# openclimatefix/predict_pv_yield

Measured on AMD Instinct MI355X. Metric: PV-site samples/sec (train step), conv3d 12->6 frames, higher is better.
Workload: dtype bf16; 1 GPU; conv3d train step (fwd + NMAE + bwd + Adam): sat [B,11,18,64,64] N(0,1), 4x Conv3d(3x3x3, 32ch) + fc 128/128/64, 128.6 M params; per_gpu_batch=32, global_batch=32, t_frames=18, parallelism=single

## Files before the change

include/pv_yield_hip.h:

```cpp
#ifndef PV_YIELD_HIP_H
#define PV_YIELD_HIP_H

#include <stddef.h>
#include <stdint.h>

#ifdef __cplusplus
extern "C" {
#endif

#define PV_ABI_VERSION 1

enum {
  PV_OK = 0,
  PV_EINVAL = -1,
  PV_ESIZE = -2,
  PV_ELAUNCH = -3
};

enum { PV_BORDER_CONSTANT = 0, PV_BORDER_REPLICATE = 1 };

enum {
  PV_U8_ROUND_DIV4 = 0,
  PV_U8_TRUNC_SCALE = 1
};
// ... 195 lines not shown
                               int transpose_flip, void* stream);

#define PV_PACK_MAX_JOBS 16
typedef struct pv_pack_job {
  const float* w;
  uint16_t* wp;
  int32_t c_out, c_in, transpose_flip;
} pv_pack_job;
int pv_conv3d_pack_weights_multi_bf16(const pv_pack_job* jobs, int32_t n_jobs, void* stream);

int pv_relu_mask_dims(int32_t h, int32_t w, int32_t* hp, int32_t* wp);
int pv_conv3d_fwd_bf16(const uint16_t* x, const uint16_t* gate, const uint16_t* wp,
                       const float* bias, uint16_t* y, const uint16_t* out_gate,
                       const uint32_t* out_gate_mask, uint32_t* relu_mask_out,
                       const pv_conv3d_dims* d, int relu, int y_ncdhw, void* stream);

int pv_conv3d_fwd_bf16_f32in(const float* x, uint16_t* xp_out, const uint16_t* wp, const float* bias, uint16_t* y,
                             uint32_t* relu_mask_out, const pv_conv3d_dims* d, int relu, void* stream);

int pv_conv3d_bwd_weight_bf16_workspace_bytes(const pv_conv3d_dims* d, size_t* bytes);
int pv_conv3d_bwd_weight_bf16(const uint16_t* x, const uint16_t* dy, const uint16_t* y_relu_mask,
                              float* dw, float* dbias, const pv_conv3d_dims* d,
                              void* workspace, size_t workspace_bytes, void* stream);
int pv_conv3d_bwd_weight_f16(const uint16_t* x, const uint16_t* dy, float* dw, float* dbias, const pv_conv3d_dims* d,
                             void* workspace, size_t workspace_bytes, void* stream);

size_t pv_conv3d_split2_weight_elems(void);
int pv_conv3d_pack_weight_split2_f16(const float* w, uint16_t* wp, float* state, int32_t c_out, int32_t c_in, void* stream);
int pv_conv3d_fwd_f16_f32out(const uint16_t* x, const uint16_t* wp, void* y, int32_t y_is_f16, const pv_conv3d_dims* d, void* stream);
int pv_conv3d_fwd_f16_f32out_covers(const pv_conv3d_dims* d);
int pv_sum3_ndhwc_to_ncdhw_f32(const float* parts, const uint16_t* p01_f16, const float* sx_state, const float* sw_state,
                               int32_t data_gradient, const float* bias, const uint16_t* gate_h, float* y, uint16_t* out_h,
                               uint16_t* out_l, float* max_state, int32_t relu, int32_t batch, int64_t vox_per_sample, void* stream);

int pv_linear_f32_skinny_covers(int32_t m, int32_t n, int64_t k);
size_t pv_linear_fwd_f32_skinny_workspace_bytes(int32_t n);
int pv_linear_fwd_f32_skinny(const float* x, const float* w, const float* bias, float* y, int32_t m, int32_t n, int64_t k, int32_t relu,
                             void* workspace, size_t workspace_bytes, void* stream);
int pv_linear_dx_f32_skinny(const float* g, const float* w, float* dx, int32_t m, int32_t n, int64_t k, void* stream);

int pv_linear_workspace_bytes(int32_t m, int32_t n, int64_t k, size_t* bytes);
int pv_linear_fwd_f32(const float* x, const float* w, const float* bias, float* y,
                      int32_t m, int32_t n, int64_t k, int relu,
                      void* workspace, size_t workspace_bytes, void* stream);
int pv_linear_bwd_f32(const float* x, const float* w, const float* dy, const float* y_relu_mask,
                      float* dx, float* dw, float* db,
// ... 175 lines not shown
```

predict_pv_yield_amd/_lib.py:

```python
import ctypes
import os
import subprocess

_PKG = os.path.dirname(os.path.abspath(__file__))
LIB_PATH = os.environ.get("PV_YIELD_LIB") or os.path.join(_PKG, "lib", "libpvyield_hip.so")
CSRC_DIR = os.path.join(_PKG, "csrc")

PV_BORDER_CONSTANT = 0
PV_BORDER_REPLICATE = 1
PV_U8_ROUND_DIV4 = 0
PV_U8_TRUNC_SCALE = 1
PV_OPTFLOW_FARNEBACK_GAUSSIAN = 256

c_i32, c_i64, c_f32, c_f64 = ctypes.c_int32, ctypes.c_int64, ctypes.c_float, ctypes.c_double
c_vp, c_sz, c_int, c_u8 = ctypes.c_void_p, ctypes.c_size_t, ctypes.c_int, ctypes.c_uint8


class FarnebackParams(ctypes.Structure):
    _fields_ = [("pyr_scale", c_f64), ("levels", c_i32), ("winsize", c_i32), ("iterations", c_i32),
                ("poly_n", c_i32), ("poly_sigma", c_f64), ("flags", c_i32)]


class Conv3dDims(ctypes.Structure):
    _fields_ = [("batch", c_i32), ("c_in", c_i32), ("c_out", c_i32), ("t_in", c_i32), ("h_in", c_i32),
# ... 59 lines not shown
    "pv_u8_stacks_from_normalised_f32": [c_vp, c_i64, c_i64, c_i64, c_i64, c_vp, c_i64, c_i32, c_i32, c_i64, c_i32, c_f32, c_vp],
    "pv_remap_bilinear_nhwc_f32": [c_vp, c_i64, c_vp, c_i64, c_i64, c_vp, c_i64, c_i64, c_i64, c_i32, c_f32, c_i32, c_i32,
                                   c_i32, c_int, c_f32, c_vp],
    "pv_normalise_i16": [c_vp, c_vp, c_sz, c_i64, c_i32, c_vp, c_vp, c_vp],
    "pv_normalise_f32": [c_vp, c_vp, c_sz, c_i64, c_i32, c_vp, c_vp, c_vp],
    "pv_bf16_cpad": [c_i32],
    "pv_pack_ncdhw_f32_to_ndhwc_bf16": [c_vp, c_vp, c_i32, c_i32, c_i32, c_i32, c_i32, c_vp],
    "pv_pack_split2_ncdhw_f32_to_ndhwc_f16": [c_vp, c_vp, c_vp, c_vp, c_i32, c_i32, c_i32, c_i32, c_i32, c_i32, c_vp],
    "pv_unpack_ndhwc_bf16_to_ncdhw_f32": [c_vp, c_vp, c_i32, c_i32, c_i32, c_i32, c_i32, c_vp],
    "pv_repack_gate_ncdhw_to_ndhwc_bf16": [c_vp, c_vp, c_vp, c_i32, c_i32, c_i32, c_i32, c_i32, c_vp],
    "pv_conv3d_packed_weight_elems": [c_i32],
    "pv_conv3d_pack_weight_bf16": [c_vp, c_vp, c_i32, c_i32, c_int, c_vp],
    "pv_relu_mask_dims": [c_i32, c_i32, c_vp, c_vp],
    "pv_ssim_mean_u8": [c_vp, c_i64, c_vp, c_i64, c_i64, c_i32, c_i32, c_f64, c_vp, c_vp],
    "pv_ssim_mean_f32": [c_vp, c_i64, c_vp, c_i64, c_i64, c_i32, c_i32, c_f64, c_vp, c_vp],
    "pv_stage_timing_begin": [],
    "pv_stage_timing_end": [c_vp, c_vp, c_vp, c_i32, c_vp],
    "pv_calibrate_copy_f32": [c_vp, c_vp, c_sz, c_vp],
    "pv_calibrate_mfma_bf16": [c_vp, c_i32, c_i32, c_vp],
    "pv_conv3d_fwd_bf16": [c_vp, c_vp, c_vp, c_vp, c_vp, c_vp, c_vp, c_vp, _PCD, c_int, c_int, c_vp],
    "pv_conv3d_fwd_bf16_f32in": [c_vp, c_vp, c_vp, c_vp, c_vp, c_vp, _PCD, c_int, c_vp],
    "pv_conv3d_bwd_weight_bf16_workspace_bytes": [_PCD, ctypes.POINTER(c_sz)],
    "pv_conv3d_bwd_weight_bf16": [c_vp, c_vp, c_vp, c_vp, c_vp, _PCD, c_vp, c_sz, c_vp],
    "pv_conv3d_bwd_weight_f16": [c_vp, c_vp, c_vp, c_vp, _PCD, c_vp, c_sz, c_vp],
    "pv_conv3d_split2_weight_elems": [],
    "pv_conv3d_pack_weight_split2_f16": [c_vp, c_vp, c_vp, c_i32, c_i32, c_vp],
    "pv_conv3d_fwd_f16_f32out": [c_vp, c_vp, c_vp, c_i32, _PCD, c_vp],
    "pv_conv3d_fwd_f16_f32out_covers": [_PCD],
    "pv_sum3_ndhwc_to_ncdhw_f32": [c_vp, c_vp, c_vp, c_vp, c_i32, c_vp, c_vp, c_vp, c_vp, c_vp, c_vp, c_i32, c_i32, c_i64, c_vp],
    "pv_linear_f32_skinny_covers": [c_i32, c_i32, c_i64],
    "pv_linear_fwd_f32_skinny_workspace_bytes": [c_i32],
    "pv_linear_fwd_f32_skinny": [c_vp, c_vp, c_vp, c_vp, c_i32, c_i32, c_i64, c_i32, c_vp, c_sz, c_vp],
    "pv_linear_dx_f32_skinny": [c_vp, c_vp, c_vp, c_i32, c_i32, c_i64, c_vp],
    "pv_linear_workspace_bytes": [c_i32, c_i32, c_i64, ctypes.POINTER(c_sz)],
    "pv_linear_fwd_f32": [c_vp, c_vp, c_vp, c_vp, c_i32, c_i32, c_i64, c_int, c_vp, c_sz, c_vp],
    "pv_linear_bwd_f32": [c_vp, c_vp, c_vp, c_vp, c_vp, c_vp, c_vp, c_i32, c_i32, c_i64, c_vp],
    "pv_linear_bf16_workspace_bytes": [c_i32, c_i32, c_i64, ctypes.POINTER(c_sz)],
    "pv_linear_fwd_bf16": [c_vp, c_vp, c_vp, c_vp, c_i32, c_i32, c_i64, c_int, c_vp, c_sz, c_vp],
    "pv_linear_bwd_bf16": [c_vp, c_vp, c_vp, c_vp, c_vp, c_vp, c_vp, c_i32, c_i32, c_i64, c_i32, c_vp],
    "pv_linear_wgrad_adam_bf16": [c_vp, c_vp, c_vp, c_vp, c_vp, c_vp, c_vp, c_i32, c_i32, c_i64, c_f64, c_f64, c_f64, c_f64,
                                  c_i32, c_vp],
    "pv_linear_wgrad_adam_f32": [c_vp, c_vp, c_vp, c_vp, c_vp, c_vp, c_i32, c_i32, c_i64, c_f64, c_f64, c_f64, c_f64, c_i32, c_vp],
    "pv_linear_wgrad_dx_adam_bf16": [c_vp, c_vp, c_vp, c_vp, c_vp, c_vp, c_vp, c_vp, c_vp, c_i32, c_i32, c_i64, c_f64, c_f64,
                                     c_f64, c_f64, c_i32, c_i32, c_i32, c_vp],
    "pv_linear_wgrad_bf16out": [c_vp, c_vp, c_vp, c_vp, c_i32, c_i32, c_i64, c_vp],
    "pv_adam_step_bf16grad": [c_vp, c_vp, c_vp, c_vp, c_vp, c_sz, c_f64, c_f64, c_f64, c_f64, c_i32, c_f32, c_vp],
# ... 166 lines not shown
```

predict_pv_yield_amd/csrc/conv3d_wgrad_bf16_v2.hip:

```cpp
#include "pv_common.h"

namespace pv {

constexpr int W2TR = 8, W2TRI = 10, W2TW = 32, W2XW = 34;
constexpr int W2_SLAB_ELEMS = 28 * 32 * 32;
constexpr uint32_t W2_INVALID = 0x40000000u;

typedef __attribute__((address_space(3))) s16x4 w2_lds_s16x4;
typedef __attribute__((address_space(3))) unsigned char* w2_lds_ptr;
typedef int w2_i32x4 __attribute__((ext_vector_type(4)));

__device__ __forceinline__ void w2_lds_dma16(uint32_t lds_addr, uint32_t voff, w2_i32x4 rsrc, uint32_t soff) {
  asm volatile("s_mov_b32 m0, %0\n\ts_nop 0\n\tbuffer_load_dwordx4 %1, %2, %3 offen lds" ::"s"(lds_addr), "v"(voff), "s"(rsrc),
               "s"(soff)
               : "memory");
}
__device__ __forceinline__ w2_i32x4 w2_rsrc(const void* base, int bytes) {
  const uintptr_t a = (uintptr_t)base;
  return (w2_i32x4){(int)(uint32_t)a, (int)((a >> 32) & 0xffffu), bytes, 0x00020000};
}

#ifdef PV_DIAG_STAMPS
__device__ unsigned long long wgrad2_diag[PV_DIAG_WAVES * PV_DIAG_SLOTS];
#endif

template <int NACC, int Q>
__device__ __forceinline__ void w2_interleave() {
  if constexpr (Q < NACC) {
    constexpr int R = 2 + 2 * NACC;
    __builtin_amdgcn_sched_group_barrier(0x008, 1, 0);
    __builtin_amdgcn_sched_group_barrier(0x100, R / NACC + (Q < R % NACC ? 1 : 0), 0);
    w2_interleave<NACC, Q + 1>();
  }
}

template <int CPAD, bool F16 = false, bool PACK12 = false>
__global__ __launch_bounds__(512, 2) void conv3d_wgrad_bf16_v2_kernel(
    const uint16_t* __restrict__ x, const uint16_t* __restrict__ dy, float* __restrict__ slabs, int t_in, int h_in, int w_in,
    int t_out, int h_out, int w_out, int pad_t, int pad_h, int pad_w, int n_colblk, int t_chunk, int rpb) {
  constexpr int NCH = CPAD / 8;
  constexpr int VPR = 16 / NCH;
  constexpr int VOXB = CPAD * 2;
  constexpr int ROWB = W2XW * VOXB;
  constexpr int SLOTB = W2TRI * ROWB;
  constexpr int XVPP = 1024 / VOXB;
  constexpr int XPIECES = (W2XW + XVPP - 1) / XVPP;
  constexpr int XTAIL_LANES = (W2XW - (XPIECES - 1) * XVPP) * NCH;
  constexpr int DROWB = W2TW * 64;
  constexpr int DSLOTB = W2TR * DROWB;
  constexpr int NXS = 5;
  __shared__ __attribute__((aligned(1024))) unsigned char lds[NXS * SLOTB + 256 + 2 * DSLOTB];
  unsigned char* lds_const = lds + NXS * SLOTB;
  unsigned char* lds_dy = lds_const + 256;

  const int tid = threadIdx.x;
  const int lane = tid & 63;
  const int wave8 = __builtin_amdgcn_readfirstlane(tid >> 6);
  const bool loader = wave8 >= 4;
  const int wave = wave8 & 3;
  const int grp = lane >> 4;
  const int qi = (lane & 15) >> 2;
  const int pi = lane & 3;
  const int hh = grp >> 1;
  const int cb = 16 * (grp & 1);

  const int h0 = blockIdx.x * rpb;
  const int b = blockIdx.z;
  const int tc0 = blockIdx.y * t_chunk;
  const int tc1 = min(tc0 + t_chunk, t_out);
  const int wg_id = (blockIdx.z * gridDim.y + blockIdx.y) * gridDim.x + blockIdx.x;
  float* slab = slabs + (size_t)wg_id * W2_SLAB_ELEMS;

  static_assert(!PACK12 || CPAD == 16, "PACK12 packs the 16-channel image");
  constexpr bool PAIRED = CPAD == 16;
  constexpr int NACC = PACK12 ? 3 : (PAIRED ? 4 : 7);
  f32x16 acc[NACC];
#pragma unroll
  for (int i = 0; i < NACC; ++i)
#pragma unroll
    for (int j = 0; j < 16; ++j) acc[i][j] = 0.f;

  const int nt = tc1 - tc0, tn = nt + 2;
  const int n_items = nt > 0 ? nt * n_colblk : 0;
  const int u_end = tn * n_colblk;
  const uint32_t lds_base = __builtin_amdgcn_readfirstlane((uint32_t)(uintptr_t)(w2_lds_ptr)lds);

  if (n_items > 0 && loader) {
    const uint32_t x_plane_b = (uint32_t)h_in * w_in * CPAD * 2u, x_row_b = (uint32_t)w_in * CPAD * 2u;
    const uint32_t d_plane_b = (uint32_t)h_out * w_out * 64u, d_row_b = (uint32_t)w_out * 64u;
    const size_t x_sample = (size_t)t_in * h_in * w_in * CPAD, d_sample = (size_t)t_out * h_out * w_out * 32;
    const void* const x_base = x + (size_t)b * x_sample;
    const void* const d_base = dy + (size_t)b * d_sample;
    const int x_bytes = (int)(x_sample * 2), d_bytes = (int)(d_sample * 2);
    uint32_t xrow_src[3];
    bool xrow_in[3];
#pragma unroll
// ... 30 lines not shown
            w2_lds_dma16(slot + (uint32_t)((wave + 4 * i) * ROWB + pc * 1024), lane_off, w2_rsrc(x_base, ok ? x_bytes : 0),
                         ok ? (uint32_t)ti * x_plane_b + xrow_src[i] : 0u);
        }
      }
    };
    auto d_slice = [&](int v_seq) {
      const int cb = v_seq / nt, t = tc0 + (v_seq - cb * nt), w0 = cb * W2TW;
      const uint32_t slot = lds_base + (uint32_t)(NXS * SLOTB + 256 + (v_seq & 1) * DSLOTB);
#pragma unroll
      for (int pc = 0; pc < 2; ++pc) {
        const int v = pc * 16 + (lane >> 2);
        const int src = (lane & 3) ^ ((v >> 2) & 3);
        const uint32_t lane_off = (w0 + v) < w_out ? (uint32_t)((w0 + v) * 32 + src * 8) * 2u : W2_INVALID;
#pragma unroll
        for (int i = 0; i < 2; ++i) {
          const bool ok = drow_in[i];
          w2_lds_dma16(slot + (uint32_t)((wave + 4 * i) * DROWB + pc * 1024), lane_off, w2_rsrc(d_base, ok ? d_bytes : 0),
                       ok ? (uint32_t)t * d_plane_b + drow_src[i] : 0u);
        }
      }
    };

    int next_u = 0;
    for (; next_u < 4 && next_u < u_end; ++next_u) x_slice(next_u);
    d_slice(0);
    for (int j = 0; j < n_items; ++j) {
      const int cb = j / nt, u0 = cb * tn + (j - cb * nt);
      __builtin_amdgcn_s_waitcnt(0x0f70);
      __syncthreads();
      if (next_u < u0 + 3) {
        for (; next_u < u0 + 3; ++next_u) x_slice(next_u);
        __builtin_amdgcn_s_waitcnt(0x0f70);
        __syncthreads();
      }
      for (; next_u <= u0 + 4 && next_u < u_end; ++next_u) x_slice(next_u);
      if (j + 1 < n_items) d_slice(j + 1);
    }
  } else if (n_items > 0) {
    if (tid < 64) reinterpret_cast<uint32_t*>(lds_const)[tid] = tid < 32 ? (F16 ? 0x3c003c00u : 0x3f803f80u) : 0u;

    int aoff[2];
#pragma unroll
    for (int s = 0; s < 2; ++s) {
      const int v = 8 * hh + 4 * s + qi;
      const int chunk = (cb + 4 * pi) >> 3;
      aoff[s] = v * 64 + ((chunk ^ ((v >> 2) & 3)) << 4) + (pi & 1) * 8;
// ... 142 lines not shown
  *n_colblk = (wo + W2TW - 1) / W2TW;
  const long long tiles = (long long)d->batch * *n_rowblk;
  int max_chunks = (to + 1) / 2;
  if (max_chunks < 1) max_chunks = 1;
  int ntc = 1;
  long long best = -1;
  for (int c = 1; c <= max_chunks && tiles * c <= 16 * 256; ++c) {
    const int tch = (to + c - 1) / c, nch = (to + tch - 1) / tch;
    const long long rounds = (tiles * nch + 255) / 256;
    const long long cost = rounds * (tch + 2);
    if (best < 0 || cost < best) best = cost, ntc = nch;
  }
  *t_chunk = (to + ntc - 1) / ntc;
  *n_tchunk = (to + *t_chunk - 1) / *t_chunk;
}

size_t wgrad_v2_workspace_bytes(const pv_conv3d_dims* d) {
  int nrb, ncb, ntc, tch, rpb;
  wgrad_v2_grid(d, &nrb, &ncb, &ntc, &tch, &rpb);
  return (size_t)d->batch * nrb * ntc * W2_SLAB_ELEMS * sizeof(float);
}

int launch_conv3d_wgrad_bf16_v2(const uint16_t* x, const uint16_t* dy, float* slabs, const pv_conv3d_dims* d, int to, int ho,
                                int wo, hipStream_t st, int* n_slabs, bool f16) {
  if (((uintptr_t)x % 16) != 0 || ((uintptr_t)dy % 16) != 0) return 1;
  int nrb, ncb, ntc, tch, rpb;
  wgrad_v2_grid(d, &nrb, &ncb, &ntc, &tch, &rpb);
  *n_slabs = d->batch * nrb * ntc;
  dim3 grid((unsigned)nrb, (unsigned)ntc, (unsigned)d->batch);
#define PV_W2(CP, HALF)                                                                                                       \
  hipLaunchKernelGGL((conv3d_wgrad_bf16_v2_kernel<CP, HALF>), grid, dim3(512), 0, st, x, dy, slabs, d->t_in, d->h_in, d->w_in, to, \
                     ho, wo, d->pad_t, d->pad_h, d->pad_w, ncb, tch, rpb)
#define PV_W2P(HALF)                                                                                                        \
  hipLaunchKernelGGL((conv3d_wgrad_bf16_v2_kernel<16, HALF, true>), grid, dim3(512), 0, st, x, dy, slabs, d->t_in, d->h_in, d->w_in, \
                     to, ho, wo, d->pad_t, d->pad_h, d->pad_w, ncb, tch, rpb)
  if (pv_bf16_cpad(d->c_in) == 16) {
    const bool pack12 = d->c_in <= 12 && !getenv("PV_WGRAD_NO_PACK12");
    if (pack12) { if (f16) PV_W2P(true); else PV_W2P(false); }
    else { if (f16) PV_W2(16, true); else PV_W2(16, false); }
  } else { if (f16) PV_W2(32, true); else PV_W2(32, false); }
#undef PV_W2P
#undef PV_W2
  return 0;
}


constexpr int WR_GROUPS = 16;
__global__ __launch_bounds__(64 * WR_GROUPS) void conv3d_wgrad_reduce_kernel(const float* __restrict__ slabs, int n_slabs,
                                                                              float* __restrict__ dw, float* __restrict__ dbias,
                                                                              int c_out, int c_in) {
  __shared__ float part[WR_GROUPS][64];
  const int lane = threadIdx.x & 63, grp = threadIdx.x >> 6;
  const int i = blockIdx.x * 64 + lane;
  float s0 = 0.f, s1 = 0.f, s2 = 0.f, s3 = 0.f;
  for (int k = grp; k < n_slabs; k += 16 * WR_GROUPS) {
    float v[16];
#pragma unroll
    for (int j = 0; j < 16; ++j) v[j] = (k + WR_GROUPS * j < n_slabs) ? slabs[(size_t)(k + WR_GROUPS * j) * W2_SLAB_ELEMS + i] : 0.f;
#pragma unroll
// ... 27 lines not shown
    u32x4 o;
#pragma unroll
    for (int j = 0; j < 4; ++j) o[j] = g[j] & (relu_pair01(a[j]) * 0xffffu);
    dst[i] = o;
  }
}

}

using namespace pv;

extern "C" {

int pv_conv3d_bwd_weight_bf16_workspace_bytes(const pv_conv3d_dims* d, size_t* bytes) {
  PV_REQUIRE(d && bytes, PV_EINVAL, "pv_conv3d_bwd_weight_bf16_workspace_bytes: null pointer");
  PV_REQUIRE(d->batch > 0 && d->t_in > 0 && d->h_in > 0 && d->w_in > 0, PV_EINVAL,
             "pv_conv3d_bwd_weight_bf16_workspace_bytes: bad dims");
  const long long to = d->t_in + 2 * d->pad_t - 2, ho = d->h_in + 2 * d->pad_h - 2, wo = d->w_in + 2 * d->pad_w - 2;
  const size_t dy_bytes = (to > 0 && ho > 0 && wo > 0) ? (size_t)d->batch * to * ho * wo * pv_bf16_cpad(d->c_out) * 2 : 0;
  *bytes = ((wgrad_v2_workspace_bytes(d) + 255) & ~(size_t)255) + dy_bytes;
  return PV_OK;
}

int pv_conv3d_bwd_weight_bf16(const uint16_t* x, const uint16_t* dy, const uint16_t* y_relu_mask, float* dw,
                              float* dbias, const pv_conv3d_dims* d, void* workspace, size_t workspace_bytes,
                              void* stream) {
  PV_REQUIRE(d && x && dy && workspace, PV_EINVAL, "pv_conv3d_bwd_weight_bf16: null pointer");
  PV_REQUIRE(d->batch > 0 && d->c_in > 0 && d->c_in <= 32 && d->c_out > 0 && d->c_out <= 32, PV_ESIZE,
             "pv_conv3d_bwd_weight_bf16: channels (%d -> %d) must be in 1..32", d->c_in, d->c_out);
  PV_REQUIRE(d->pad_t >= 0 && d->pad_t <= 2 && d->pad_h >= 0 && d->pad_h <= 2 && d->pad_w >= 0 && d->pad_w <= 2,
             PV_EINVAL, "pv_conv3d_bwd_weight_bf16: padding must be 0..2");
  const int to = d->t_in + 2 * d->pad_t - 2, ho = d->h_in + 2 * d->pad_h - 2, wo = d->w_in + 2 * d->pad_w - 2;
  PV_REQUIRE(to > 0 && ho > 0 && wo > 0, PV_ESIZE, "pv_conv3d_bwd_weight_bf16: input smaller than the kernel");
  PV_REQUIRE(d->batch <= 65535, PV_ESIZE, "pv_conv3d_bwd_weight_bf16: batch too large for grid.z");
  PV_REQUIRE((size_t)d->t_in * d->h_in * d->w_in * 64 <= 0x40000000ull, PV_ESIZE,
             "pv_conv3d_bwd_weight_bf16: one sample exceeds 1 GiB (buffer-addressing limit of this kernel)");
  const size_t slab_bytes = (wgrad_v2_workspace_bytes(d) + 255) & ~(size_t)255;
  PV_REQUIRE(workspace_bytes >= wgrad_v2_workspace_bytes(d), PV_ESIZE, "pv_conv3d_bwd_weight_bf16: workspace too small");
  PV_REQUIRE(((uintptr_t)x % 16) == 0 && ((uintptr_t)dy % 16) == 0 && ((uintptr_t)workspace % 16) == 0, PV_EINVAL,
             "pv_conv3d_bwd_weight_bf16: x, dy and the workspace must be 16-byte aligned");
  hipStream_t st = as_stream(stream);
  if (y_relu_mask) {
    const size_t n = (size_t)d->batch * to * ho * wo * pv_bf16_cpad(d->c_out);
    PV_REQUIRE(workspace_bytes >= slab_bytes + n * 2, PV_ESIZE,
               "pv_conv3d_bwd_weight_bf16: a gate needs room for the gated copy of dY behind the slabs (workspace_bytes query)");
    PV_REQUIRE(((uintptr_t)y_relu_mask % 16) == 0, PV_EINVAL, "pv_conv3d_bwd_weight_bf16: the gate must be 16-byte aligned");
    uint16_t* gated = reinterpret_cast<uint16_t*>(static_cast<char*>(workspace) + slab_bytes);
    hipLaunchKernelGGL(wgrad_gate_copy_kernel, dim3(stream_grid(n / 8, 256)), dim3(256), 0, st,
                       reinterpret_cast<const u32x4*>(dy), reinterpret_cast<const u32x4*>(y_relu_mask),
                       reinterpret_cast<u32x4*>(gated), n / 8);
    dy = gated;
  }
  int n2 = 0;
  PV_REQUIRE(launch_conv3d_wgrad_bf16_v2(x, dy, (float*)workspace, d, to, ho, wo, st, &n2, false) == 0, PV_EINVAL,
             "pv_conv3d_bwd_weight_bf16: x and dy must be 16-byte aligned");
  hipLaunchKernelGGL(conv3d_wgrad_reduce_kernel, dim3(W2_SLAB_ELEMS / 64), dim3(64 * WR_GROUPS), 0, st, (const float*)workspace, n2,
                     dw, dbias, d->c_out, d->c_in);
  return check_launch("pv_conv3d_bwd_weight_bf16");
}

int pv_conv3d_bwd_weight_f16(const uint16_t* x, const uint16_t* dy, float* dw, float* dbias, const pv_conv3d_dims* d,
                             void* workspace, size_t workspace_bytes, void* stream) {
  PV_REQUIRE(d && x && dy && workspace, PV_EINVAL, "pv_conv3d_bwd_weight_f16: null pointer");
  PV_REQUIRE(d->batch > 0 && d->c_in > 0 && d->c_in <= 32 && d->c_out > 0 && d->c_out <= 32, PV_ESIZE,
             "pv_conv3d_bwd_weight_f16: channels (%d -> %d) must be in 1..32", d->c_in, d->c_out);
  PV_REQUIRE(d->pad_t >= 0 && d->pad_t <= 2 && d->pad_h >= 0 && d->pad_h <= 2 && d->pad_w >= 0 && d->pad_w <= 2,
             PV_EINVAL, "pv_conv3d_bwd_weight_f16: padding must be 0..2");
  const int to = d->t_in + 2 * d->pad_t - 2, ho = d->h_in + 2 * d->pad_h - 2, wo = d->w_in + 2 * d->pad_w - 2;
  PV_REQUIRE(to > 0 && ho > 0 && wo > 0, PV_ESIZE, "pv_conv3d_bwd_weight_f16: input smaller than the kernel");
  PV_REQUIRE(d->batch <= 65535, PV_ESIZE, "pv_conv3d_bwd_weight_f16: batch too large for grid.z");
  PV_REQUIRE((size_t)d->t_in * d->h_in * d->w_in * 64 <= 0x40000000ull, PV_ESIZE,
             "pv_conv3d_bwd_weight_f16: one sample exceeds 1 GiB (buffer-addressing limit of this kernel)");
  PV_REQUIRE(workspace_bytes >= wgrad_v2_workspace_bytes(d), PV_ESIZE, "pv_conv3d_bwd_weight_f16: workspace too small");
  hipStream_t st = as_stream(stream);
  int n2 = 0;
  PV_REQUIRE(launch_conv3d_wgrad_bf16_v2(x, dy, (float*)workspace, d, to, ho, wo, st, &n2, true) == 0, PV_EINVAL,
             "pv_conv3d_bwd_weight_f16: x and dy must be 16-byte aligned");
  hipLaunchKernelGGL(conv3d_wgrad_reduce_kernel, dim3(W2_SLAB_ELEMS / 64), dim3(64 * WR_GROUPS), 0, st, (const float*)workspace, n2,
                     dw, dbias, d->c_out, d->c_in);
  return check_launch("pv_conv3d_bwd_weight_f16");
}
// ... 9 lines not shown
```

predict_pv_yield_amd/csrc/linear_bf16.hip:

```cpp
#include "pv_common.h"
#include <string.h>

namespace pv {

template <int MT>
__global__ __launch_bounds__(256) void linear_fwd_bf16_kernel(const uint16_t* __restrict__ x,
                                                               const uint16_t* __restrict__ w,
                                                               float* __restrict__ partial, int m, int n,
                                                               long long k, int kblocks_per_wg) {
  const int lane = threadIdx.x & 63;
  const int wave = threadIdx.x >> 6;
  const int r = lane & 31, hh = lane >> 5;
  const int nt = blockIdx.y * 4 + wave;
  const long long total_kb = (k + 63) / 64;
  const long long kb0 = (long long)blockIdx.x * kblocks_per_wg;
  long long kb1 = kb0 + kblocks_per_wg;
  if (kb1 > total_kb) kb1 = total_kb;

  int wrow = nt * 32 + r;
  if (wrow > n - 1) wrow = n - 1;
  const uint16_t* wp = w + (size_t)wrow * k + 32 * hh;
  const uint16_t* xp[MT];
#pragma unroll
  for (int mt = 0; mt < MT; ++mt) {
// ... 1018 lines not shown
      }
    }
    __syncthreads();
    for (int i = tid; i < 128 * (WB_KC / 8); i += 256) {
      const int row = i >> 4, c = i & 15;
      if (row < n && k0 + 8 * c < k)
        *reinterpret_cast<u32x4*>(dw + (size_t)row * k + k0 + 8 * c) = *reinterpret_cast<const u32x4*>(ot + row * WB_OS + 8 * c);
    }
  }
}

__global__ __launch_bounds__(256) void gate_bf16_by_relu_kernel(uint16_t* __restrict__ dx, const uint16_t* __restrict__ x, size_t n8) {
  for (size_t i = (size_t)blockIdx.x * blockDim.x + threadIdx.x; i < n8; i += (size_t)gridDim.x * blockDim.x) {
    u32x4 d = reinterpret_cast<const u32x4*>(dx)[i];
    const u32x4 xv = reinterpret_cast<const u32x4*>(x)[i];
#pragma unroll
    for (int q = 0; q < 4; ++q) d[q] &= __builtin_bit_cast(uint32_t, __builtin_bit_cast(u16x2_t, relu_pair01(xv[q])) * (u16x2_t){0xffff, 0xffff});
    reinterpret_cast<u32x4*>(dx)[i] = d;
  }
}

constexpr int V3_KC = 128;

template <int MB>
__global__ __launch_bounds__(256) void linear_fwd_bf16_v3_kernel(const uint16_t* __restrict__ x, const uint16_t* __restrict__ w,
                                                                  float* __restrict__ partial, int m, int n, long long k,
                                                                  int n_tiles, int tiles_per_wg) {
  constexpr int V3_ROWS = 128 + 32 * MB, V3_TILEB = V3_ROWS * 256, LOADS = V3_ROWS / 16, V3_STAGES = MB <= 2 ? 3 : 2;
  __shared__ __attribute__((aligned(1024))) unsigned char ring[V3_STAGES * V3_TILEB];
  const int lane = threadIdx.x & 63;
  const int wave = __builtin_amdgcn_readfirstlane(threadIdx.x >> 6);
  const int r = lane & 31, hh = lane >> 5;
  const int t0 = blockIdx.x * tiles_per_wg;
  const int t1 = t0 + tiles_per_wg < n_tiles ? t0 + tiles_per_wg : n_tiles;
  if (t0 >= t1) return;
  constexpr uint32_t INVALID = 0xfffffff0u;
  const __amdgpu_buffer_rsrc_t wrsrc = __builtin_amdgcn_make_buffer_rsrc((void*)w, 0, (int)((size_t)n * k * 2), 0x00020000);
  const __amdgpu_buffer_rsrc_t xrsrc = __builtin_amdgcn_make_buffer_rsrc((void*)x, 0, (int)((size_t)m * k * 2), 0x00020000);
  const int srow = lane >> 4, spos = lane & 15;
  auto load_tile = [&](int t) {
    unsigned char* dst = ring + (t % V3_STAGES) * V3_TILEB;
    const long long k0 = (long long)t * V3_KC;
    typedef __attribute__((address_space(3))) void* lds_ptr_t;
#pragma unroll
    for (int i = 0; i < LOADS; ++i) {
      const int blk = wave + 4 * i;
      const int row = 4 * blk + srow;
      const int c = (spos - row) & 15;
      const bool c_ok = k0 + c * 8 < k;
      if (blk < 32) {
        const uint32_t off = (c_ok && row < n) ? (uint32_t)(((size_t)row * k + k0 + c * 8) * 2) : INVALID;
        __builtin_amdgcn_raw_ptr_buffer_load_lds(wrsrc, (lds_ptr_t)(dst + blk * 1024), 16, off, 0, 0, 0);
      } else {
        const int xr = row - 128;
        const uint32_t off = (c_ok && xr < m) ? (uint32_t)(((size_t)xr * k + k0 + c * 8) * 2) : INVALID;
        __builtin_amdgcn_raw_ptr_buffer_load_lds(xrsrc, (lds_ptr_t)(dst + blk * 1024), 16, off, 0, 0, 0);
      }
    }
  };
  f32x16 acc[MB];
#pragma unroll
  for (int q = 0; q < MB; ++q)
#pragma unroll
    for (int j = 0; j < 16; ++j) acc[q][j] = 0.f;
  int pos[V3_KC / 16];
#pragma unroll
  for (int ks = 0; ks < V3_KC / 16; ++ks) pos[ks] = ((2 * ks + hh + r) & 15) * 16;
  const int a_row = (128 + r) * 256, b_row = (wave * 32 + r) * 256;

  load_tile(t0);
  if (V3_STAGES == 3 && t0 + 1 < t1) load_tile(t0 + 1);
  for (int t = t0; t < t1; ++t) {
    if (V3_STAGES == 3 && t + 1 < t1) __builtin_amdgcn_s_waitcnt(0x0f70 | (LOADS & 15));
    else __builtin_amdgcn_s_waitcnt(0x0f70);
    __syncthreads();
    if (t + V3_STAGES - 1 < t1) load_tile(t + V3_STAGES - 1);
    const unsigned char* tile = ring + (t % V3_STAGES) * V3_TILEB;
    if (wave * 32 < n) {
#pragma unroll
      for (int ks = 0; ks < V3_KC / 16; ++ks) {
        const bf16x8 b = *reinterpret_cast<const bf16x8*>(tile + b_row + pos[ks]);
#pragma unroll
        for (int q = 0; q < MB; ++q) {
          const bf16x8 a = *reinterpret_cast<const bf16x8*>(tile + a_row + q * (32 * 256) + pos[ks]);
          acc[q] = __builtin_amdgcn_mfma_f32_32x32x16_bf16(a, b, acc[q], 0, 0, 0);
        }
      }
    }
  }
  const int col = wave * 32 + r;
  if (col < n) {
    float* dst = partial + (size_t)blockIdx.x * m * n + col;
#pragma unroll
    for (int q = 0; q < MB; ++q)
#pragma unroll
      for (int j = 0; j < 16; ++j) {
// ... 293 lines not shown
```

predict_pv_yield_amd/functional.py:

```python
import ctypes

import torch

from . import hip_ops as K
from ._lib import check, current_stream_ptr, get_lib, ptr


LINEAR_F32_GEMM_K = 1 << 16
F32_PENDING_MAX_ROWS = 1024


def exact_f32() -> bool:
    import os
    return bool(os.environ.get("PV_EXACT_F32"))


class LinearF32(torch.autograd.Function):
    @staticmethod
    def forward(ctx, x, weight, bias, relu):
        x = x.contiguous()
        if (not exact_f32() and x.dtype == torch.float32 and weight.is_contiguous()
                and K.linear_f32_skinny_covers(x.shape[0], weight.shape[0], x.shape[1])):
            y = K.linear_fwd_f32_skinny(x, weight, bias.contiguous() if bias is not None else None, relu)
        else:
# ... 119 lines not shown
        if y_ncdhw:
            dy = K.repack_gate_ncdhw_to_ndhwc_bf16(dy, None if _take_pregated(dy) else y)
            gate = None
        elif dy_pregated == "ask":
            gate = None if _take_pregated(dy) else y
        elif dy_pregated:
            gate = None
        else:
            gate = y
        dw, db = K.conv3d_bwd_weight_bf16(xp, dy, gate, c_in, c_out, padding)
        dx = None
        if ctx.needs_input_grad[0]:
            wpt = packed_conv_weight(weight, True)
            pad_b = tuple(2 - p for p in padding)
            out_gate = xp if (x_is_relu_output and xp.shape[-1] == 32) else None
            gate_mask = x_relu_mask if (out_gate is not None and x_relu_mask is not None and x_relu_mask.numel()) else None
            dx = K.conv3d_fwd_bf16(dy, gate, wpt, None, c_out, c_in, pad_b, relu=False, y_ncdhw=False, out_gate=out_gate,
                                   out_gate_mask=gate_mask)
            if K.bf16_cpad(c_in) != 32:
                dx = dx[..., : K.bf16_cpad(c_in)].contiguous()
        return dx, dw, (db if has_bias else None), None, None, None, None, None, None, None, None


class Conv3dFirstLayerBF16(torch.autograd.Function):

    @staticmethod
    def forward(ctx, x, weight, bias, padding, relu, dy_pregated, want_relu_mask):
        wp = packed_conv_weight(weight, False)
        c_out, c_in = weight.shape[0], weight.shape[1]
        need_bwd = ctx.needs_input_grad[1] or ctx.needs_input_grad[2]
        want_relu_mask = bool(want_relu_mask and relu and need_bwd)
        out = K.conv3d_fwd_bf16_f32in(x.contiguous(), wp, bias.contiguous() if bias is not None else None, c_out, padding,
                                      relu, want_packed=need_bwd, want_relu_mask=want_relu_mask)
        y, xp = out[0], out[1]
        mask = out[2] if want_relu_mask else torch.empty(0, dtype=torch.int32, device=y.device)
        ctx.save_for_backward(xp, weight, y if relu else None)
        ctx.cfg = (c_in, c_out, padding, bias is not None, dy_pregated)
        ctx.mark_non_differentiable(mask)
        ctx.set_materialize_grads(False)
        return y, mask

    @staticmethod
    def backward(ctx, dy, _dmask):
        xp, weight, y = ctx.saved_tensors
        c_in, c_out, padding, has_bias, dy_pregated = ctx.cfg
        gate = None if dy_pregated else y
        dw, db = K.conv3d_bwd_weight_bf16(xp, dy.contiguous(), gate, c_in, c_out, padding)
        return None, dw, (db if has_bias else None), None, None, None, None


def conv3d_first_layer_bf16(x, weight, bias, padding=(0, 0, 0), relu=True, dy_pregated=False, want_relu_mask=False):
    y, mask = Conv3dFirstLayerBF16.apply(x, weight, bias, tuple(padding), relu, dy_pregated, want_relu_mask)
    return (y, mask) if want_relu_mask else y


def bf16_shadow_of(weight: torch.Tensor) -> torch.Tensor:
    work = getattr(weight, "_pv_shadow_work", None)
    if work is not None:
        work.wait()
        weight._pv_shadow_work = None
    shadow = getattr(weight, "_pv_bf16_shadow", None)
    version = getattr(weight, "_pv_bf16_shadow_version", None)
    if shadow is None or shadow.device != weight.device or version != weight._version:
        shadow = torch.empty(weight.shape, dtype=torch.bfloat16, device=weight.device)
        check(get_lib().pv_cast_f32_to_bf16(ptr(weight.detach()), ptr(shadow), weight.numel(), current_stream_ptr()),
              "pv_cast_f32_to_bf16")
        weight._pv_bf16_shadow = shadow
        weight._pv_bf16_shadow_version = weight._version
    return shadow

# ... 431 lines not shown
```

predict_pv_yield_amd/hip_ops.py:

```python
import ctypes
from typing import Optional, Sequence

import numpy as np
import torch

from . import _lib
from ._lib import (Conv3dDims, Conv3dGeom, FarnebackParams, PV_BORDER_CONSTANT, PV_BORDER_REPLICATE,
                   PV_OPTFLOW_FARNEBACK_GAUSSIAN, check, current_stream_ptr, get_lib, ptr, require_cuda)

c_i32, c_i64, c_f32, c_f64, c_sz = ctypes.c_int32, ctypes.c_int64, ctypes.c_float, ctypes.c_double, ctypes.c_size_t


def u8_from_10bit(x: torch.Tensor, mode: int = 0, return_flag: bool = False):
    require_cuda(x)
    out = torch.empty(x.shape, dtype=torch.uint8, device=x.device)
    flag = torch.zeros(1, dtype=torch.int32, device=x.device)
    lib = get_lib()
    if x.dtype == torch.int16:
        fn = lib.pv_u8_from_10bit_i16
    elif x.dtype == torch.float32:
        fn = lib.pv_u8_from_10bit_f32
    else:
        raise TypeError(f"u8_from_10bit: int16 or float32 expected, got {x.dtype}")
    check(fn(ptr(x), ptr(out), x.numel(), mode, ptr(flag), current_stream_ptr()), "pv_u8_from_10bit")
# ... 494 lines not shown
    d = conv_dims(b, c_in, c_out, t, h, w, padding)
    to, ho, wo = d.out_shape()
    y = torch.empty((b, to, ho, wo, 32), dtype=torch.bfloat16, device=x.device)
    xp = torch.empty((b, t, h, w, 16), dtype=torch.bfloat16, device=x.device) if want_packed else None
    mask = torch.empty(relu_mask_shape(b, to, ho, wo), dtype=torch.int32, device=x.device) if want_relu_mask else None
    check(get_lib().pv_conv3d_fwd_bf16_f32in(ptr(x), ptr(xp), ptr(wp), ptr(bias), ptr(y), ptr(mask), ctypes.byref(d),
                                             int(relu), current_stream_ptr()), "pv_conv3d_fwd_bf16_f32in")
    return (y, xp, mask) if want_relu_mask else (y, xp)


def conv3d_bwd_weight_bf16(x: torch.Tensor, dy: torch.Tensor, y_mask: Optional[torch.Tensor], c_in: int, c_out: int,
                           padding=(0, 0, 0)):
    require_cuda(x, dy, y_mask)
    b, t, h, w, cpad = x.shape
    d = conv_dims(b, c_in, c_out, t, h, w, padding)
    need = c_sz(0)
    lib = get_lib()
    check(lib.pv_conv3d_bwd_weight_bf16_workspace_bytes(ctypes.byref(d), ctypes.byref(need)), "wgrad workspace")
    ws = _workspace("wgrad", need.value, x.device)
    dw = torch.empty((c_out, c_in, 3, 3, 3), dtype=torch.float32, device=x.device)
    db = torch.empty(c_out, dtype=torch.float32, device=x.device)
    check(lib.pv_conv3d_bwd_weight_bf16(ptr(x), ptr(dy), ptr(y_mask), ptr(dw), ptr(db), ctypes.byref(d), ptr(ws),
                                        ws.numel(), current_stream_ptr()), "pv_conv3d_bwd_weight_bf16")
    return dw, db


def linear_fwd_f32(x, weight, bias, relu=False):
    require_cuda(x, weight, bias)
    m, k = x.shape
    n = weight.shape[0]
    need = c_sz(0)
    lib = get_lib()
    check(lib.pv_linear_workspace_bytes(m, n, k, ctypes.byref(need)), "pv_linear_workspace_bytes")
    ws = _workspace("linear", need.value, x.device)
    y = torch.empty((m, n), dtype=torch.float32, device=x.device)
    check(lib.pv_linear_fwd_f32(ptr(x), ptr(weight), ptr(bias), ptr(y), m, n, k, int(relu), ptr(ws), ws.numel(),
                                current_stream_ptr()), "pv_linear_fwd_f32")
    return y


LINEAR_F32_SKINNY = True


def linear_f32_skinny_covers(m: int, n: int, k: int) -> bool:
    return LINEAR_F32_SKINNY and bool(get_lib().pv_linear_f32_skinny_covers(m, n, k))

# ... 1261 lines not shown
```

Before: 20760 samples/s.

## Read f32 input directly in first-layer wgrad and deepen linear v3 pipeline

The first conv layer no longer writes a packed bf16 copy of the f32 satellite input during forward. The weight-gradient kernel instead gains an XF32 path that loads the f32 NCDHW input with buffer loads and converts it to bf16 in LDS, keeping loads in flight across slices. Separately, the skinny bf16 linear kernel uses a 4-stage ring with inline-asm LDS DMA for MB==1 and a wider vmcnt wait. The first part trades the forward write plus backward reread of the bf16 image for strided f32 reads (twice the bytes) and in-kernel conversion inside wgrad.

```diff
diff --git a/include/pv_yield_hip.h b/include/pv_yield_hip.h
--- a/include/pv_yield_hip.h
+++ b/include/pv_yield_hip.h
@@ -241,6 +241,9 @@
 int pv_conv3d_bwd_weight_bf16(const uint16_t* x, const uint16_t* dy, const uint16_t* y_relu_mask,
                               float* dw, float* dbias, const pv_conv3d_dims* d,
                               void* workspace, size_t workspace_bytes, void* stream);
+int pv_conv3d_bwd_weight_bf16_f32in(const float* x, const uint16_t* dy, const uint16_t* y_relu_mask,
+                                    float* dw, float* dbias, const pv_conv3d_dims* d,
+                                    void* workspace, size_t workspace_bytes, void* stream);
 int pv_conv3d_bwd_weight_f16(const uint16_t* x, const uint16_t* dy, float* dw, float* dbias, const pv_conv3d_dims* d,
                              void* workspace, size_t workspace_bytes, void* stream);
 
diff --git a/predict_pv_yield_amd/_lib.py b/predict_pv_yield_amd/_lib.py
--- a/predict_pv_yield_amd/_lib.py
+++ b/predict_pv_yield_amd/_lib.py
@@ -105,6 +105,7 @@
     "pv_conv3d_fwd_bf16_f32in": [c_vp, c_vp, c_vp, c_vp, c_vp, c_vp, _PCD, c_int, c_vp],
     "pv_conv3d_bwd_weight_bf16_workspace_bytes": [_PCD, ctypes.POINTER(c_sz)],
     "pv_conv3d_bwd_weight_bf16": [c_vp, c_vp, c_vp, c_vp, c_vp, _PCD, c_vp, c_sz, c_vp],
+    "pv_conv3d_bwd_weight_bf16_f32in": [c_vp, c_vp, c_vp, c_vp, c_vp, _PCD, c_vp, c_sz, c_vp],
     "pv_conv3d_bwd_weight_f16": [c_vp, c_vp, c_vp, c_vp, _PCD, c_vp, c_sz, c_vp],
     "pv_conv3d_split2_weight_elems": [],
     "pv_conv3d_pack_weight_split2_f16": [c_vp, c_vp, c_vp, c_i32, c_i32, c_vp],
diff --git a/predict_pv_yield_amd/csrc/conv3d_wgrad_bf16_v2.hip b/predict_pv_yield_amd/csrc/conv3d_wgrad_bf16_v2.hip
--- a/predict_pv_yield_amd/csrc/conv3d_wgrad_bf16_v2.hip
+++ b/predict_pv_yield_amd/csrc/conv3d_wgrad_bf16_v2.hip
@@ -34,10 +34,10 @@
   }
 }
 
-template <int CPAD, bool F16 = false, bool PACK12 = false>
+template <int CPAD, bool F16 = false, bool PACK12 = false, bool XF32 = false>
 __global__ __launch_bounds__(512, 2) void conv3d_wgrad_bf16_v2_kernel(
     const uint16_t* __restrict__ x, const uint16_t* __restrict__ dy, float* __restrict__ slabs, int t_in, int h_in, int w_in,
-    int t_out, int h_out, int w_out, int pad_t, int pad_h, int pad_w, int n_colblk, int t_chunk, int rpb) {
+    int t_out, int h_out, int w_out, int pad_t, int pad_h, int pad_w, int n_colblk, int t_chunk, int rpb, int c_in) {
   constexpr int NCH = CPAD / 8;
   constexpr int VPR = 16 / NCH;
   constexpr int VOXB = CPAD * 2;
@@ -72,6 +72,7 @@
   float* slab = slabs + (size_t)wg_id * W2_SLAB_ELEMS;
 
   static_assert(!PACK12 || CPAD == 16, "PACK12 packs the 16-channel image");
+  static_assert(!XF32 || (PACK12 && !F16), "the f32-input loaders write the bf16 image of at most 12 channels");
   constexpr bool PAIRED = CPAD == 16;
   constexpr int NACC = PACK12 ? 3 : (PAIRED ? 4 : 7);
   f32x16 acc[NACC];
@@ -148,6 +149,86 @@
     };
 
     int next_u = 0;
+    if constexpr (XF32) {
+      constexpr int XF_LOADS = 12;
+      const int task = wave * 23 + lane;
+      const bool has = lane < 23 && task < W2TRI * 9;
+      const int f_row = has ? task / 9 : 0, f_quad = has ? task - 9 * f_row : 0;
+      const size_t f32_sample_b = (size_t)c_in * t_in * h_in * w_in * 4;
+      const __amdgpu_buffer_rsrc_t xrsrc = __builtin_amdgcn_make_buffer_rsrc(
+          (void*)(reinterpret_cast<const unsigned char*>(x) + (size_t)b * f32_sample_b), 0, (int)f32_sample_b, 0x00020000);
+      const uint32_t f_plane_b = (uint32_t)t_in * h_in * w_in * 4u, f_slice_b = (uint32_t)h_in * w_in * 4u;
+      const int f_hi = h0 - pad_h + f_row;
+      const uint32_t f_row_off = (has && (unsigned)f_hi < (unsigned)h_in && f_row < rpb + 2) ? (uint32_t)f_hi * (uint32_t)w_in * 4u : W2_INVALID;
+      uint32_t f_ch_off[XF_LOADS];
+#pragma unroll
+      for (int ch = 0; ch < XF_LOADS; ++ch) f_ch_off[ch] = ch < c_in ? (uint32_t)ch * f_plane_b : W2_INVALID;
+      auto x_load = [&](int u, f32x4 (&st)[XF_LOADS]) {
+        const int cb = u / tn, s = tc0 + (u - cb * tn);
+        const int ti = s - pad_t, wi = cb * W2TW + 4 * f_quad;
+        const uint32_t toff = (unsigned)ti < (unsigned)t_in ? (uint32_t)ti * f_slice_b : W2_INVALID;
+        const uint32_t lane_off = wi < w_in ? f_row_off + (uint32_t)wi * 4u : W2_INVALID;
+#pragma unroll
+        for (int ch = 0; ch < XF_LOADS; ++ch)
+          st[ch] = __builtin_bit_cast(f32x4, __builtin_amdgcn_raw_buffer_load_b128(xrsrc, lane_off + f_ch_off[ch], toff, 0));
+      };
+      auto x_store = [&](int u, const f32x4 (&st)[XF_LOADS]) {
+        if (!has) return;
+        unsigned char* row = lds + (u % NXS) * SLOTB + f_row * ROWB;
+#pragma unroll
+        for (int q = 0; q < 4; ++q) {
+          const int v = 4 * f_quad + q;
+          if (v >= W2XW) continue;
+#pragma unroll
+          for (int sc = 0; sc < 2; ++sc) {
+            u32x4 c;
+#pragma unroll
+            for (int e = 0; e < 4; ++e)
+              c[e] = 8 * sc + 2 * e < XF_LOADS ? pack_bf16_pair(st[(8 * sc + 2 * e) % XF_LOADS][q], st[(8 * sc + 2 * e + 1) % XF_LOADS][q]) : 0u;
+            *reinterpret_cast<u32x4*>(row + v * VOXB + ((sc ^ ((v / VPR) % NCH)) << 4)) = c;
+          }
+        }
+      };
+      f32x4 st[4][XF_LOADS];
+#pragma unroll
+      for (int q = 0; q < 4; ++q)
+        if (q < u_end) x_load(q, st[q]);
+      d_slice(0);
+#pragma unroll
+      for (int q = 0; q < 4; ++q)
+        if (q < u_end) x_store(q, st[q]);
+      next_u = u_end < 4 ? u_end : 4;
+      bool in_flight = next_u < u_end;
+      if (in_flight) x_load(next_u, st[0]);
+      for (int j = 0; j < n_items; ++j) {
+        const int cb = j / nt, u0 = cb * tn + (j - cb * nt);
+        if (in_flight) __builtin_amdgcn_s_waitcnt(0x0f70 | XF_LOADS);
+        else __builtin_amdgcn_s_waitcnt(0x0f70);
+        __syncthreads();
+        if (next_u < u0 + 3) {
+          for (; next_u < u0 + 3; ) {
+            x_store(next_u, st[0]);
+            in_flight = ++next_u < u_end;
+            if (in_flight) x_load(next_u, st[0]);
+          }
+          if (in_flight) __builtin_amdgcn_s_waitcnt(0x0f70 | XF_LOADS);
+          else __builtin_amdgcn_s_waitcnt(0x0f70);
+          __syncthreads();
+        }
+        bool dy_asked = j + 1 >= n_items;
+        for (; next_u <= u0 + 4 && next_u < u_end; ) {
+          x_store(next_u, st[0]);
+          if (!dy_asked) d_slice(j + 1), dy_asked = true;
+          in_flight = ++next_u < u_end;
+          if (in_flight) x_load(next_u, st[0]);
+        }
+        if (!dy_asked) {
+          d_slice(j + 1);
+          if (in_flight) __builtin_amdgcn_s_waitcnt(0x0f70);
+        }
+      }
+      return;
+    }
     for (; next_u < 4 && next_u < u_end; ++next_u) x_slice(next_u);
     d_slice(0);
     for (int j = 0; j < n_items; ++j) {
@@ -336,19 +417,23 @@
 }
 
 int launch_conv3d_wgrad_bf16_v2(const uint16_t* x, const uint16_t* dy, float* slabs, const pv_conv3d_dims* d, int to, int ho,
-                                int wo, hipStream_t st, int* n_slabs, bool f16) {
+                                int wo, hipStream_t st, int* n_slabs, bool f16, bool x_f32 = false) {
   if (((uintptr_t)x % 16) != 0 || ((uintptr_t)dy % 16) != 0) return 1;
+  if (x_f32 && (f16 || d->c_in > 12 || d->pad_w != 0 || d->w_in % 4 != 0)) return 1;
   int nrb, ncb, ntc, tch, rpb;
   wgrad_v2_grid(d, &nrb, &ncb, &ntc, &tch, &rpb);
   *n_slabs = d->batch * nrb * ntc;
   dim3 grid((unsigned)nrb, (unsigned)ntc, (unsigned)d->batch);
 #define PV_W2(CP, HALF)                                                                                                       \
   hipLaunchKernelGGL((conv3d_wgrad_bf16_v2_kernel<CP, HALF>), grid, dim3(512), 0, st, x, dy, slabs, d->t_in, d->h_in, d->w_in, to, \
-                     ho, wo, d->pad_t, d->pad_h, d->pad_w, ncb, tch, rpb)
+                     ho, wo, d->pad_t, d->pad_h, d->pad_w, ncb, tch, rpb, d->c_in)
 #define PV_W2P(HALF)                                                                                                        \
   hipLaunchKernelGGL((conv3d_wgrad_bf16_v2_kernel<16, HALF, true>), grid, dim3(512), 0, st, x, dy, slabs, d->t_in, d->h_in, d->w_in, \
-                     to, ho, wo, d->pad_t, d->pad_h, d->pad_w, ncb, tch, rpb)
-  if (pv_bf16_cpad(d->c_in) == 16) {
+                     to, ho, wo, d->pad_t, d->pad_h, d->pad_w, ncb, tch, rpb, d->c_in)
+  if (x_f32) {
+    hipLaunchKernelGGL((conv3d_wgrad_bf16_v2_kernel<16, false, true, true>), grid, dim3(512), 0, st, x, dy, slabs, d->t_in, d->h_in,
+                       d->w_in, to, ho, wo, d->pad_t, d->pad_h, d->pad_w, ncb, tch, rpb, d->c_in);
+  } else if (pv_bf16_cpad(d->c_in) == 16) {
     const bool pack12 = d->c_in <= 12 && !getenv("PV_WGRAD_NO_PACK12");
     if (pack12) { if (f16) PV_W2P(true); else PV_W2P(false); }
     else { if (f16) PV_W2(16, true); else PV_W2(16, false); }
@@ -422,10 +507,13 @@
   return PV_OK;
 }
 
-int pv_conv3d_bwd_weight_bf16(const uint16_t* x, const uint16_t* dy, const uint16_t* y_relu_mask, float* dw,
-                              float* dbias, const pv_conv3d_dims* d, void* workspace, size_t workspace_bytes,
-                              void* stream) {
+static int bwd_weight_bf16(const void* x, bool x_f32, const uint16_t* dy, const uint16_t* y_relu_mask, float* dw, float* dbias,
+                           const pv_conv3d_dims* d, void* workspace, size_t workspace_bytes, void* stream) {
   PV_REQUIRE(d && x && dy && workspace, PV_EINVAL, "pv_conv3d_bwd_weight_bf16: null pointer");
+  if (x_f32)
+    PV_REQUIRE(d->c_in > 0 && d->c_in <= 12 && d->pad_w == 0 && d->w_in % 4 == 0, PV_ESIZE,
+               "pv_conv3d_bwd_weight_bf16_f32in: built for 1..12 input channels, pad_w == 0 and w_in %% 4 == 0 (got %d, %d, %d): "
+               "other shapes take pv_conv3d_bwd_weight_bf16 on the bf16 image", d->c_in, d->pad_w, d->w_in);
   PV_REQUIRE(d->batch > 0 && d->c_in > 0 && d->c_in <= 32 && d->c_out > 0 && d->c_out <= 32, PV_ESIZE,
              "pv_conv3d_bwd_weight_bf16: channels (%d -> %d) must be in 1..32", d->c_in, d->c_out);
   PV_REQUIRE(d->pad_t >= 0 && d->pad_t <= 2 && d->pad_h >= 0 && d->pad_h <= 2 && d->pad_w >= 0 && d->pad_w <= 2,
@@ -452,11 +540,23 @@
     dy = gated;
   }
   int n2 = 0;
-  PV_REQUIRE(launch_conv3d_wgrad_bf16_v2(x, dy, (float*)workspace, d, to, ho, wo, st, &n2, false) == 0, PV_EINVAL,
-             "pv_conv3d_bwd_weight_bf16: x and dy must be 16-byte aligned");
+  PV_REQUIRE(launch_conv3d_wgrad_bf16_v2((const uint16_t*)x, dy, (float*)workspace, d, to, ho, wo, st, &n2, false, x_f32) == 0,
+             PV_EINVAL, "pv_conv3d_bwd_weight_bf16: x and dy must be 16-byte aligned");
   hipLaunchKernelGGL(conv3d_wgrad_reduce_kernel, dim3(W2_SLAB_ELEMS / 64), dim3(64 * WR_GROUPS), 0, st, (const float*)workspace, n2,
                      dw, dbias, d->c_out, d->c_in);
-  return check_launch("pv_conv3d_bwd_weight_bf16");
+  return check_launch(x_f32 ? "pv_conv3d_bwd_weight_bf16_f32in" : "pv_conv3d_bwd_weight_bf16");
+}
+
+int pv_conv3d_bwd_weight_bf16(const uint16_t* x, const uint16_t* dy, const uint16_t* y_relu_mask, float* dw,
+                              float* dbias, const pv_conv3d_dims* d, void* workspace, size_t workspace_bytes,
+                              void* stream) {
+  return bwd_weight_bf16(x, false, dy, y_relu_mask, dw, dbias, d, workspace, workspace_bytes, stream);
+}
+
+int pv_conv3d_bwd_weight_bf16_f32in(const float* x, const uint16_t* dy, const uint16_t* y_relu_mask, float* dw,
+                                    float* dbias, const pv_conv3d_dims* d, void* workspace, size_t workspace_bytes,
+                                    void* stream) {
+  return bwd_weight_bf16(x, true, dy, y_relu_mask, dw, dbias, d, workspace, workspace_bytes, stream);
 }
 
 int pv_conv3d_bwd_weight_f16(const uint16_t* x, const uint16_t* dy, float* dw, float* dbias, const pv_conv3d_dims* d,
diff --git a/predict_pv_yield_amd/csrc/linear_bf16.hip b/predict_pv_yield_amd/csrc/linear_bf16.hip
--- a/predict_pv_yield_amd/csrc/linear_bf16.hip
+++ b/predict_pv_yield_amd/csrc/linear_bf16.hip
@@ -1064,11 +1064,22 @@
 
 constexpr int V3_KC = 128;
 
+typedef int v3_i32x4 __attribute__((ext_vector_type(4)));
+__device__ __forceinline__ void v3_lds_dma16(uint32_t lds_addr, uint32_t voff, v3_i32x4 rsrc) {
+  asm volatile("s_mov_b32 m0, %0\n\ts_nop 0\n\tbuffer_load_dwordx4 %1, %2, 0 offen lds" ::"s"(lds_addr), "v"(voff), "s"(rsrc)
+               : "memory");
+}
+__device__ __forceinline__ v3_i32x4 v3_rsrc(const void* base, size_t bytes) {
+  const uintptr_t a = (uintptr_t)base;
+  return (v3_i32x4){(int)(uint32_t)a, (int)((a >> 32) & 0xffffu), (int)(uint32_t)bytes, 0x00020000};
+}
+
 template <int MB>
 __global__ __launch_bounds__(256) void linear_fwd_bf16_v3_kernel(const uint16_t* __restrict__ x, const uint16_t* __restrict__ w,
                                                                   float* __restrict__ partial, int m, int n, long long k,
                                                                   int n_tiles, int tiles_per_wg) {
-  constexpr int V3_ROWS = 128 + 32 * MB, V3_TILEB = V3_ROWS * 256, LOADS = V3_ROWS / 16, V3_STAGES = MB <= 2 ? 3 : 2;
+  constexpr int V3_ROWS = 128 + 32 * MB, V3_TILEB = V3_ROWS * 256, LOADS = V3_ROWS / 16, V3_STAGES = MB == 1 ? 4 : (MB == 2 ? 3 : 2);
+  static_assert(V3_STAGES * V3_TILEB <= 160 * 1024 && 2 * LOADS < 64, "ring within a CU's LDS, vmcnt within its 6 bits");
   __shared__ __attribute__((aligned(1024))) unsigned char ring[V3_STAGES * V3_TILEB];
   const int lane = threadIdx.x & 63;
   const int wave = __builtin_amdgcn_readfirstlane(threadIdx.x >> 6);
@@ -1080,8 +1091,12 @@
   const __amdgpu_buffer_rsrc_t wrsrc = __builtin_amdgcn_make_buffer_rsrc((void*)w, 0, (int)((size_t)n * k * 2), 0x00020000);
   const __amdgpu_buffer_rsrc_t xrsrc = __builtin_amdgcn_make_buffer_rsrc((void*)x, 0, (int)((size_t)m * k * 2), 0x00020000);
   const int srow = lane >> 4, spos = lane & 15;
+  typedef __attribute__((address_space(3))) unsigned char* lds_byte_ptr_t;
+  const uint32_t ring_addr = __builtin_amdgcn_readfirstlane((uint32_t)(uintptr_t)(lds_byte_ptr_t)ring);
+  const v3_i32x4 wdesc = v3_rsrc(w, (size_t)n * k * 2), xdesc = v3_rsrc(x, (size_t)m * k * 2);
   auto load_tile = [&](int t) {
     unsigned char* dst = ring + (t % V3_STAGES) * V3_TILEB;
+    const uint32_t dst_addr = ring_addr + (uint32_t)((t % V3_STAGES) * V3_TILEB);
     const long long k0 = (long long)t * V3_KC;
     typedef __attribute__((address_space(3))) void* lds_ptr_t;
 #pragma unroll
@@ -1092,11 +1107,13 @@
       const bool c_ok = k0 + c * 8 < k;
       if (blk < 32) {
         const uint32_t off = (c_ok && row < n) ? (uint32_t)(((size_t)row * k + k0 + c * 8) * 2) : INVALID;
-        __builtin_amdgcn_raw_ptr_buffer_load_lds(wrsrc, (lds_ptr_t)(dst + blk * 1024), 16, off, 0, 0, 0);
+        if constexpr (MB == 1) v3_lds_dma16(dst_addr + blk * 1024, off, wdesc);
+        else __builtin_amdgcn_raw_ptr_buffer_load_lds(wrsrc, (lds_ptr_t)(dst + blk * 1024), 16, off, 0, 0, 0);
       } else {
         const int xr = row - 128;
         const uint32_t off = (c_ok && xr < m) ? (uint32_t)(((size_t)xr * k + k0 + c * 8) * 2) : INVALID;
-        __builtin_amdgcn_raw_ptr_buffer_load_lds(xrsrc, (lds_ptr_t)(dst + blk * 1024), 16, off, 0, 0, 0);
+        if constexpr (MB == 1) v3_lds_dma16(dst_addr + blk * 1024, off, xdesc);
+        else __builtin_amdgcn_raw_ptr_buffer_load_lds(xrsrc, (lds_ptr_t)(dst + blk * 1024), 16, off, 0, 0, 0);
       }
     }
   };
@@ -1110,10 +1127,13 @@
   for (int ks = 0; ks < V3_KC / 16; ++ks) pos[ks] = ((2 * ks + hh + r) & 15) * 16;
   const int a_row = (128 + r) * 256, b_row = (wave * 32 + r) * 256;
 
-  load_tile(t0);
-  if (V3_STAGES == 3 && t0 + 1 < t1) load_tile(t0 + 1);
+#pragma unroll
+  for (int i = 0; i < V3_STAGES - 1; ++i)
+    if (t0 + i < t1) load_tile(t0 + i);
   for (int t = t0; t < t1; ++t) {
-    if (V3_STAGES == 3 && t + 1 < t1) __builtin_amdgcn_s_waitcnt(0x0f70 | (LOADS & 15));
+    const int newer = t1 - 1 - t;
+    if (V3_STAGES >= 4 && newer >= 2) __builtin_amdgcn_s_waitcnt(0x0f70 | ((2 * LOADS) & 15) | (((2 * LOADS) >> 4) << 14));
+    else if (V3_STAGES >= 3 && newer >= 1) __builtin_amdgcn_s_waitcnt(0x0f70 | (LOADS & 15));
     else __builtin_amdgcn_s_waitcnt(0x0f70);
     __syncthreads();
     if (t + V3_STAGES - 1 < t1) load_tile(t + V3_STAGES - 1);
diff --git a/predict_pv_yield_amd/functional.py b/predict_pv_yield_amd/functional.py
--- a/predict_pv_yield_amd/functional.py
+++ b/predict_pv_yield_amd/functional.py
@@ -1,4 +1,5 @@
 import ctypes
+import os
 
 import torch
 
@@ -165,6 +166,10 @@
         return dx, dw, (db if has_bias else None), None, None, None, None, None, None, None, None
 
 
+def first_layer_keeps_bf16_copy() -> bool:
+    return bool(os.environ.get("PV_CONV_FIRST_BF16_COPY"))
+
+
 class Conv3dFirstLayerBF16(torch.autograd.Function):
 
     @staticmethod
@@ -173,11 +178,14 @@
         c_out, c_in = weight.shape[0], weight.shape[1]
         need_bwd = ctx.needs_input_grad[1] or ctx.needs_input_grad[2]
         want_relu_mask = bool(want_relu_mask and relu and need_bwd)
-        out = K.conv3d_fwd_bf16_f32in(x.contiguous(), wp, bias.contiguous() if bias is not None else None, c_out, padding,
-                                      relu, want_packed=need_bwd, want_relu_mask=want_relu_mask)
+        x = x.contiguous()
+        from_f32 = need_bwd and not first_layer_keeps_bf16_copy() and K.conv3d_bwd_weight_bf16_f32in_covers(c_in, x.shape[4], padding)
+        out = K.conv3d_fwd_bf16_f32in(x, wp, bias.contiguous() if bias is not None else None, c_out, padding,
+                                      relu, want_packed=need_bwd and not from_f32, want_relu_mask=want_relu_mask)
         y, xp = out[0], out[1]
         mask = out[2] if want_relu_mask else torch.empty(0, dtype=torch.int32, device=y.device)
-        ctx.save_for_backward(xp, weight, y if relu else None)
+        ctx.save_for_backward(x if from_f32 else xp, weight, y if relu else None)
+        ctx.from_f32 = from_f32
         ctx.cfg = (c_in, c_out, padding, bias is not None, dy_pregated)
         ctx.mark_non_differentiable(mask)
         ctx.set_materialize_grads(False)
@@ -188,7 +196,10 @@
         xp, weight, y = ctx.saved_tensors
         c_in, c_out, padding, has_bias, dy_pregated = ctx.cfg
         gate = None if dy_pregated else y
-        dw, db = K.conv3d_bwd_weight_bf16(xp, dy.contiguous(), gate, c_in, c_out, padding)
+        if ctx.from_f32:
+            dw, db = K.conv3d_bwd_weight_bf16_f32in(xp, dy.contiguous(), gate, c_out, padding)
+        else:
+            dw, db = K.conv3d_bwd_weight_bf16(xp, dy.contiguous(), gate, c_in, c_out, padding)
         return None, dw, (db if has_bias else None), None, None, None, None
 
 
diff --git a/predict_pv_yield_amd/hip_ops.py b/predict_pv_yield_amd/hip_ops.py
--- a/predict_pv_yield_amd/hip_ops.py
+++ b/predict_pv_yield_amd/hip_ops.py
@@ -540,6 +540,28 @@
     db = torch.empty(c_out, dtype=torch.float32, device=x.device)
     check(lib.pv_conv3d_bwd_weight_bf16(ptr(x), ptr(dy), ptr(y_mask), ptr(dw), ptr(db), ctypes.byref(d), ptr(ws),
                                         ws.numel(), current_stream_ptr()), "pv_conv3d_bwd_weight_bf16")
+    return dw, db
+
+
+def conv3d_bwd_weight_bf16_f32in_covers(c_in: int, w: int, padding=(0, 0, 0)) -> bool:
+    return 0 < c_in <= 12 and w % 4 == 0 and tuple(padding)[2] == 0
+
+
+def conv3d_bwd_weight_bf16_f32in(x: torch.Tensor, dy: torch.Tensor, y_mask: Optional[torch.Tensor], c_out: int,
+                                 padding=(0, 0, 0)):
+    require_cuda(x, dy, y_mask)
+    if x.dtype != torch.float32 or x.dim() != 5 or not x.is_contiguous():
+        raise TypeError("conv3d_bwd_weight_bf16_f32in: x must be a contiguous f32 [B,C,T,H,W] tensor")
+    b, c_in, t, h, w = x.shape
+    d = conv_dims(b, c_in, c_out, t, h, w, padding)
+    need = c_sz(0)
+    lib = get_lib()
+    check(lib.pv_conv3d_bwd_weight_bf16_workspace_bytes(ctypes.byref(d), ctypes.byref(need)), "wgrad workspace")
+    ws = _workspace("wgrad", need.value, x.device)
+    dw = torch.empty((c_out, c_in, 3, 3, 3), dtype=torch.float32, device=x.device)
+    db = torch.empty(c_out, dtype=torch.float32, device=x.device)
+    check(lib.pv_conv3d_bwd_weight_bf16_f32in(ptr(x), ptr(dy), ptr(y_mask), ptr(dw), ptr(db), ctypes.byref(d), ptr(ws),
+                                              ws.numel(), current_stream_ptr()), "pv_conv3d_bwd_weight_bf16_f32in")
     return dw, db
 
 
```

Result: no change. 20970 samples/s (median of 6 runs) (+1.0%).
